# soham97/mellow

Hardware: AMD Instinct MI355X
Metric: audio-pair responses/sec (v0 167M, 2x10s clips, max_len=64, greedy) (higher is better)
Workload: dtype f32 (encoder/prefill GEMM operands split EXACTLY into 3 bf16 terms, 6 bf16 MFMA products per fp32 product, f32 accumulate: fp32-accurate, parity suite green; mel included, the STFT is an fp32 FFT; attentions and decode on exact fp32 MFMA / VALU)

## Files before the change

mellow_amd/csrc/build.py:

```python
#!/usr/bin/env python3
from __future__ import annotations

import argparse
import concurrent.futures as cf
import os
import subprocess
import sys

HERE = os.path.dirname(os.path.abspath(__file__))
PKG = os.path.dirname(HERE)
LIBDIR = os.path.join(PKG, "lib")
OBJDIR = os.path.join(HERE, "build")
LIB = os.path.join(LIBDIR, "libmellow_hip.so")
SOURCES = ["gemm_f32.hip", "gemm_fp8.hip", "gemm_bf16x3.hip", "decode.hip", "prefill_attn.hip", "encoder.hip", "stft_fft.hip", "sample.hip", "score.hip", "beam.hip", "engine.cpp", "engine_weights.cpp", "engine_encoder.cpp", "engine_lm.cpp", "engine_generate.cpp", "engine_dev.cpp"]
HEADERS = ["common.h", "kernels.h", "gemm_epilogue.h", "prefill_attn_f32.inc", "engine_internal.h", os.path.join("..", "..", "include", "mellow_hip.h")]
ARCH = "gfx950"
FLAGS = (["-DMELLOW_KDEBUG"] if os.environ.get("MELLOW_KDEBUG") else []) + os.environ.get("MELLOW_EXTRA_FLAGS", "").split() + ["-O3", "-std=c++17", "-fPIC", "-fvisibility=hidden", f"--offload-arch={ARCH}", "-Wall", "-Wno-unused-function",
         "-Wno-unused-variable", "-x", "hip"]


def _hipcc():
    for c in (os.environ.get("HIPCC"), "/opt/rocm/bin/hipcc", "hipcc"):
        if c and (os.path.isabs(c) and os.path.exists(c) or not os.path.isabs(c)):
            return c
    raise RuntimeError("hipcc not found")


def _stale(target, deps):
    if not os.path.exists(target):
        return True
    t = os.path.getmtime(target)
    return any(os.path.getmtime(d) > t for d in deps)


VGPR_FORM = ["-mllvm", "-amdgpu-mfma-vgpr-form=1"]
FILE_FLAGS = {name: VGPR_FORM for name in os.environ.get("MELLOW_VGPR_FORM_FILES", "gemm_bf16x3.hip gemm_fp8.hip prefill_attn.hip encoder.hip").split()}
KERNARG_PRELOAD = [] if os.environ.get("MELLOW_KERNARG_PRELOAD", "14") == "0" else ["-mllvm", "-amdgpu-kernarg-preload-count=" + os.environ.get("MELLOW_KERNARG_PRELOAD", "14")]
FILE_FLAGS["decode.hip"] = FILE_FLAGS.get("decode.hip", []) + KERNARG_PRELOAD


def build(force=False, verbose=False, out=None, objdir=None):
    lib = os.path.abspath(out) if out else LIB
    objdir = os.path.abspath(objdir) if objdir else OBJDIR
    os.makedirs(os.path.dirname(lib), exist_ok=True)
    os.makedirs(objdir, exist_ok=True)
    hipcc = _hipcc()
    hdrs = [os.path.join(HERE, h) for h in HEADERS] + [os.path.abspath(__file__)]
    jobs = []
    objs = []
    for src in SOURCES:
        sp = os.path.join(HERE, src)
        op = os.path.join(objdir, src + ".o")
        objs.append(op)
        if force or _stale(op, [sp] + hdrs):
            jobs.append((sp, op))

    def cc(job):
        sp, op = job
        cmd = [hipcc] + FLAGS + FILE_FLAGS.get(os.path.basename(sp), []) + ["-c", sp, "-o", op]
        if verbose:
            print(" ".join(cmd), flush=True)
        r = subprocess.run(cmd, capture_output=True, text=True)
        return sp, r

    with cf.ThreadPoolExecutor(max_workers=max(1, min(len(jobs), os.cpu_count() or 1))) as ex:
        for sp, r in ex.map(cc, jobs):
            if r.returncode != 0:
                sys.stderr.write(r.stdout + r.stderr)
                raise RuntimeError(f"hipcc failed on {sp}")
            if verbose and r.stderr.strip():
                sys.stderr.write(r.stderr)
    if force or jobs or _stale(lib, objs):
        cmd = [hipcc, "-shared", "-fPIC", f"--offload-arch={ARCH}", "-o", lib] + objs
        if verbose:
            print(" ".join(cmd), flush=True)
        r = subprocess.run(cmd, capture_output=True, text=True)
        if r.returncode != 0:
            sys.stderr.write(r.stdout + r.stderr)
            raise RuntimeError("link failed")
    return lib


if __name__ == "__main__":
    ap = argparse.ArgumentParser()
    ap.add_argument("--force", action="store_true")
    ap.add_argument("--verbose", action="store_true")
    ap.add_argument("--out", metavar="PATH", help="write the library here instead of mellow_amd/lib/libmellow_hip.so")
    ap.add_argument("--objdir", metavar="DIR", help="object cache of this build instead of mellow_amd/csrc/build/")
    a = ap.parse_args()
# ... 2 lines not shown
```

mellow_amd/csrc/common.h:

```cpp
#pragma once
#include <hip/hip_runtime.h>
#include <stdint.h>

namespace mellow {

typedef float f32x16 __attribute__((ext_vector_type(16)));
typedef float f32x4 __attribute__((ext_vector_type(4)));

#define MELLOW_WAVE 64

template <int CTRL>
__device__ __forceinline__ float dpp_mov(float v) {
    return __int_as_float(__builtin_amdgcn_update_dpp(0, __float_as_int(v), CTRL, 0xF, 0xF, true));
}
__device__ __forceinline__ float row16_sum(float v) {
    v += dpp_mov<0xB1>(v);
    v += dpp_mov<0x4E>(v);
    v += dpp_mov<0x141>(v);
    v += dpp_mov<0x140>(v);
    return v;
}
__device__ __forceinline__ float row16_max(float v) {
    v = fmaxf(v, dpp_mov<0xB1>(v));
    v = fmaxf(v, dpp_mov<0x4E>(v));
// ... 119 lines not shown
}

__device__ __forceinline__ int64_t amx_slot(int64_t m, int s, int j, int h, int KT64) {
    return (((((m >> 7) * KT64 + s) * 4 + ((m >> 5) & 3)) * 2 + j) * 64) + (m & 31) + 32 * h;
}
__device__ __forceinline__ int64_t amx_scale_byte(int64_t m, int s, int j, int KQ) {
    return (((((m >> 7) * KQ + (s >> 2)) * 4 + ((m >> 5) & 3)) * 64) + (m & 31) + 32 * j) * 4 + (s & 3);
}
__device__ __forceinline__ int mx8_exponent(float amax) {
    const uint32_t b = __float_as_uint(amax * (1.0f / 448.0f));
    int e = (int)((b >> 23) & 0xFF) + ((b & 0x7FFFFF) ? 1 : 0);
    e = e < 1 ? 1 : (e > 253 ? 253 : e);
    return amax > 0.f ? e : 127;
}
__device__ __forceinline__ float mx8_inverse(int e) { return __uint_as_float((uint32_t)(254 - e) << 23); }
__device__ __forceinline__ int mx8_pack4(float a, float b, float c, float d) {
    int w = 0;
    w = __builtin_amdgcn_cvt_pk_fp8_f32(a, b, w, false);
    w = __builtin_amdgcn_cvt_pk_fp8_f32(c, d, w, true);
    return w;
}
__device__ __forceinline__ void amx_store_block(i32x4* img, uint8_t* sc, int64_t m, int kb, int KT64, int KQ, const float (&v)[16], int h) {
    float amax = 0.f;
#pragma unroll
    for (int i = 0; i < 16; ++i) amax = fmaxf(amax, fabsf(v[i]));
    amax = half_max(amax);
    const int e = mx8_exponent(amax);
    const float inv = mx8_inverse(e);
    int w[4];
#pragma unroll
    for (int g = 0; g < 4; ++g) w[g] = mx8_pack4(v[4 * g] * inv, v[4 * g + 1] * inv, v[4 * g + 2] * inv, v[4 * g + 3] * inv);
    auto r0 = __builtin_amdgcn_permlane32_swap((uint32_t)w[0], (uint32_t)w[2], false, false);
    auto r1 = __builtin_amdgcn_permlane32_swap((uint32_t)w[1], (uint32_t)w[3], false, false);
    const int s = kb >> 1, j = kb & 1;
    img[amx_slot(m, s, j, h, KT64)] = i32x4{(int)r0[0], (int)r0[1], (int)r1[0], (int)r1[1]};
    if (h == 0) sc[amx_scale_byte(m, s, j, KQ)] = (uint8_t)e;
}

__device__ __forceinline__ void amx_store16(i32x4* img, uint8_t* sc, int64_t m, int kb, int KT64, int KQ, const float (&y)[16], int h) {
    float amax = 0.f;
#pragma unroll
    for (int i = 0; i < 16; ++i) amax = fmaxf(amax, fabsf(y[i]));
    amax = half_max(amax);
    const int e = mx8_exponent(amax);
    const float inv = mx8_inverse(e);
    i32x4 w;
#pragma unroll
    for (int q = 0; q < 4; ++q) w[q] = mx8_pack4(y[4 * q] * inv, y[4 * q + 1] * inv, y[4 * q + 2] * inv, y[4 * q + 3] * inv);
    const int s = kb >> 1, j = kb & 1;
    img[amx_slot(m, s, j, h, KT64)] = w;
    if (h == 0) sc[amx_scale_byte(m, s, j, KQ)] = (uint8_t)e;
}

__device__ __forceinline__ int xcd_remap(int b, int nb) {
    const int q = nb >> 3, r = nb & 7, x = b & 7;
    const int base = (x < r) ? x * (q + 1) : r * (q + 1) + (x - r) * q;
    return base + (b >> 3);
}

}
```

mellow_amd/csrc/engine.cpp:

```cpp
#include "engine_internal.h"

static thread_local std::string g_err;
int fail(const char* fmt, ...) {
    char buf[1024];
    va_list ap;
    va_start(ap, fmt);
    vsnprintf(buf, sizeof(buf), fmt, ap);
    va_end(ap);
    g_err = buf;
    return 1;
}
int ensure(mellow_engine* e, mellow_engine::Buf& b, size_t floats) {
    if (b.cap >= floats) return 0;
    if (b.p) HIPCHK(hipFree(b.p));
    b.p = nullptr;
    b.cap = 0;
    HIPCHK(hipMalloc(&b.p, floats * sizeof(float)));
    b.cap = floats;
    return 0;
}
int dev_alloc(mellow_engine* e, float** out, size_t floats) {
    const size_t bytes = (floats * sizeof(float) + 4095) / 4096 * 4096;
    if (!e->arena) {
        const size_t want = (size_t)(e->opt.arena_mb < 0 ? 0 : e->opt.arena_mb) << 20;
// ... 291 lines not shown
    *yes = h[2] < h[1];
    return 0;
}
int ensure_prefill_streams(mellow_engine* e) {
    if (e->n_forks > 0 || e->parent) return 0;
    if (e->streams_probed) {
        if (++e->probe_backoff < 16) { e->prefill_parts = e->prefill_parts_ok; return 0; }
        e->streams_probed = false;
        e->probe_backoff = 0;
        e->prefill_parts = e->prefill_parts_want;
    }
    int nh = e->prefill_parts < 1 ? 1 : (e->prefill_parts > 4 ? 4 : e->prefill_parts);
    for (int h = 1; h < nh; ++h) {
        if (e->stream2[h - 1]) continue;
        bool ok = false;
        for (int attempt = 0; attempt < 8 && !ok; ++attempt) {
            hipStream_t st = nullptr;
            HIPCHK(hipStreamCreateWithFlags(&st, hipStreamNonBlocking));
            int rc = streams_overlap(e, e->stream, st, &ok);
            for (int k = 1; k < h && ok && !rc; ++k) rc = streams_overlap(e, e->stream2[k - 1], st, &ok);
            if (rc) { hipStreamDestroy(st); return rc; }
            if (ok) e->stream2[h - 1] = st; else hipStreamDestroy(st);
        }
        if (!ok) {
            e->prefill_parts_want = e->prefill_parts;
            e->prefill_parts = e->prefill_parts_ok = h;
            e->streams_probed = true;
            break;
        }
    }
    return 0;
}
struct OptDesc { const char* key; const char* dflt; bool answers; const char* what; };
static const OptDesc kOptions[] = {
    {"prefill_split", "2", false, "f32x3: parts of the split LM prefill (1..4); bit-identical for every value"},
    {"prefill_fuse_norm", "1", true, "f32x3: norm-free LM prefill (GEMM epilogues emit split output + RMS partials); 0 = a normalisation launch per GEMM input"},
    {"decode_fuse", "1", true, "down projection of layer l fused with q/k/v of layer l + 1 through the load-time product W'Wd; 0 = five launches per layer"},
    {"decode_fuse_max_rb", "1", true, "largest number of 32-row blocks that runs the fused down + q/k/v launch on fp32 weights"},
    {"splitk", "8", true, "f32x3 encoder: largest split count of the split-K launches (0 = never split; a summation order)"},
    {"enc_apb", "0x1CC", false, "f32x3 encoder: Swin stages whose producers hand over pre-split (bit st, 4 + st, 8 + st); bit-identical"},
    {"graph", "1", false, "decode steps as hipGraph replays (0 = eager launches)"},
    {"fp8_decode", "1", true, "fp8 mode: e4m3 weights in the decode kernels"},
    {"fp8_prefill", "1", true, "fp8 mode: e4m3 GEMMs in encoder + LM prefill"},
    {"fp8_decode_act", "1", true, "fp8 mode: e4m3 activations in the decode GEMM kernels (fp8 matrix pipe)"},
    {"fp8_kv16", "1", true, "fp8 mode: bf16 shadow of the K/V pages for the decode step"},
    {"fp8_attn_bf16", "1", true, "fp8 mode: q / k / v stored once as bf16 (LM: bf16 K/V pages + bf16-once prefill attention; Swin: bf16 q/k/v rows into the exact window attention); 0 = fp32 q/k/v, the 3-way split attention"},
    {"decode_x3", "7", true, "f32x3: mask of decode GEMM launches on the bf16 pipe (1 lm_head, 2 gate/up, 4 fused down + q/k/v)"},
    {"decode_x3_min_rb", "2", true, "f32x3: fewest 32-row blocks at which the layer launches take their f32x3 forms"},
    {"x3_stft", "1", true, "f32x3: STFT / mel GEMMs on the split kernel (0 = exact fp32 kernel)"},
    {"stft_fft", "1", true, "f32x3: STFT as a 1024-point FFT when the checkpoint's conv weights are the windowed DFT basis"},
    {"x3_apb", "1", true, "f32x3 LM prefill: producers hand over pre-split, GEMMs staged by LDS-DMA (0 = register-staged kernel on fp32 activations)"},
    {"x3_attn", "1", true, "f32x3: prefill attention on exact bf16 splits (0 = exact fp32 MFMA kernel)"},
    {"x3w", "1", false, "f32x3: K = 96 GEMMs on the weight-stationary persistent kernel; bit-identical"},
    {"row_migration", "1", false, "reference-semantics loop, B > 32: rows still running are packed into the lowest 32-row blocks; tokens unchanged"},
    {"arena_mb", "3400", false, "size of the weight arena in MiB (before the first tensor is loaded)"},
};
static const OptDesc* find_opt(const char* key) {
    for (const auto& o : kOptions)
        if (!strcmp(o.key, key)) return &o;
    return nullptr;
}
static long opt_val(const mellow_engine* e, const char* key) {
    auto it = e->opt.given.find(key);
    return strtol(it != e->opt.given.end() ? it->second.c_str() : find_opt(key)->dflt, nullptr, 0);
}
int apply_options(mellow_engine* e) {
    const int mode = e->opt.mode;
    e->prefill_parts = (int)opt_val(e, "prefill_split");
    e->opt.prefill_fuse_norm = opt_val(e, "prefill_fuse_norm") != 0;
    e->opt.decode_fuse = opt_val(e, "decode_fuse") != 0;
    e->opt.dec_fuse_max_rb = (int)opt_val(e, "decode_fuse_max_rb");
    e->opt.sk_max = (int)opt_val(e, "splitk");
    e->opt.enc_apb_stages = (int)opt_val(e, "enc_apb");
    e->use_graph = opt_val(e, "graph") != 0;
    e->opt.x3_stft = opt_val(e, "x3_stft") != 0;
    e->opt.stft_fft = opt_val(e, "stft_fft") != 0 && e->opt.x3_stft;
    e->opt.x3_apb = opt_val(e, "x3_apb") != 0;
    e->opt.x3_attn = opt_val(e, "x3_attn") != 0;
    e->opt.x3w = opt_val(e, "x3w") != 0;
    e->opt.row_migration = opt_val(e, "row_migration") != 0;
    e->opt.arena_mb = (int)opt_val(e, "arena_mb");
    e->opt.fp8 = mode == MELLOW_PRECISION_FP8;
    e->opt.fp8_decode = e->opt.fp8 && opt_val(e, "fp8_decode") != 0;
    e->opt.fp8_decode_act = e->opt.fp8_decode && opt_val(e, "fp8_decode_act") != 0;
    e->opt.fp8_prefill = opt_val(e, "fp8_prefill") != 0;
    e->opt.fp8_attn_bf16 = opt_val(e, "fp8_attn_bf16") != 0;
    e->opt.kv16 = e->opt.fp8_decode && opt_val(e, "fp8_kv16") != 0;
    e->opt.f32x3_terms = mode == MELLOW_PRECISION_F32X3 ? 6 : 0;
    e->opt.dec_x3 = mode == MELLOW_PRECISION_F32X3 ? ((int)opt_val(e, "decode_x3") & DEC_X3_ALL) : 0;
    e->opt.dec_x3_min_rb = (int)opt_val(e, "decode_x3_min_rb") < 1 ? 1 : (int)opt_val(e, "decode_x3_min_rb");
    return 0;
}

extern "C" {

int mellow_engine_set_option(mellow_engine_t* e, const char* key, const char* value) {
    if (!e || !key || !value) return fail("null argument");
    if (e->finalized) return fail("options must be set before mellow_engine_finalize");
    const OptDesc* o = find_opt(key);
    if (!o) return fail("unknown option \"%s\" (mellow_engine_describe lists them)", key);
    char* end = nullptr;
    const long v = strtol(value, &end, 0);
    if (end == value || *end) return fail("option \"%s\": \"%s\" is not an integer", key, value);
    if (!strcmp(key, "prefill_split") && (v < 1 || v > 4)) return fail("option prefill_split must be 1..4");
    if (!strcmp(key, "arena_mb") && e->arena) return fail("option arena_mb must be set before the first tensor is loaded");
    e->opt.given[key] = value;
    return apply_options(e);
}

int64_t mellow_engine_describe(mellow_engine_t* e, char* buf, int64_t capacity) {
    if (!e) return -1;
    std::string s = "{\"abi\": [" + std::to_string(MELLOW_ABI_VERSION) + ", " + std::to_string(MELLOW_ABI_MINOR) + "], \"precision\": \"";
    s += e->opt.mode == MELLOW_PRECISION_F32 ? "f32" : e->opt.mode == MELLOW_PRECISION_FP8 ? "fp8" : "f32x3";
    s += "\", \"reads_environment\": false, \"finalized\": ";
    s += e->finalized ? "true" : "false";
    s += ", \"stft_is_fft\": ";
    s += e->w.fft_win ? "true" : "false";
    s += ", \"non_default\": [";
    bool first = true;
    for (const auto& o : kOptions)
        if (opt_val(e, o.key) != strtol(o.dflt, nullptr, 0)) { s += std::string(first ? "" : ", ") + "\"" + o.key + "\""; first = false; }
    s += "], \"options\": {";
    first = true;
    for (const auto& o : kOptions) {
        s += std::string(first ? "" : ", ") + "\"" + o.key + "\": {\"value\": " + std::to_string(opt_val(e, o.key)) + ", \"default\": " +
             std::to_string(strtol(o.dflt, nullptr, 0)) + ", \"changes_answers\": " + (o.answers ? "true" : "false") + "}";
        first = false;
    }
    s += "}}";
    if (buf && capacity > (int64_t)s.size()) memcpy(buf, s.c_str(), s.size() + 1);
    return (int64_t)s.size() + 1;
}
// ... 99 lines not shown
```

mellow_amd/csrc/engine_encoder.cpp:

```cpp
#include "engine_internal.h"

static void with_splitk(mellow_engine* e, GemmArgs& g) {
    if (!e->sk_enable || e->opt.sk_max < 2 || !e->sk_ws.p) return;
    g.sk_ws = e->sk_ws.p;
    g.sk_tiles = 256;
    g.sk_max = e->opt.sk_max;
}
int run_gemm(mellow_engine* e, const GemmArgs& a) {
    const bool x3_stft = e->opt.x3_stft;
    if (e->opt.f32x3_terms && a.K % 16 == 0 &&
        ((a.a_mode == A_PLAIN && (a.epi == EPI_LINEAR || a.epi == EPI_SWIGLU || a.epi == EPI_QKV_ROPE || a.epi == EPI_QKV_ROPE_AT)) || (x3_stft && a.K >= 192))) {
        auto it = e->w.bf_w.find(a.Wp);
        if (it != e->w.bf_w.end()) {
            GemmArgs g = a;
            g.W8 = reinterpret_cast<const uint8_t*>(it->second);
            with_splitk(e, g);
            ProfScope ps(e, PF_GEMM, gemm_flops(a), 0.0);
            ps.r.M = a.M; ps.r.N = a.Nw; ps.r.K = a.K; ps.r.epi = a.epi + 200;
            launch_gemm_bf16x3_fused(g, e->stream);
            return 0;
        }
    }
    if (e->opt.fp8 && e->opt.fp8_prefill && a.a_mode == A_PLAIN && (a.epi == EPI_LINEAR || a.epi == EPI_SWIGLU || a.epi == EPI_QKV_ROPE)) {
        auto it = e->w.fp8_w.find(a.Wp);
// ... 52 lines not shown
    hipStream_t s = e->stream;
    struct SkScope {
        mellow_engine* e;
        ~SkScope() { e->sk_enable = false; }
    } sk_scope{e};
    if (e->opt.f32x3_terms && e->opt.sk_max >= 2) {
        CHK(ensure(e, e->sk_ws, (size_t)512 * 16384));
        e->sk_enable = e->sk_ws.p != nullptr;
    }
    const int frames = (int)(n_samples / kHop) + 1;
    const int64_t plen = n_samples + kNfft;
    const int M = n * frames;
    CHK(ensure(e, e->wpad, (size_t)n * plen));
    CHK(ensure(e, e->power, (size_t)M * 544));
    CHK(ensure(e, e->logmel, (size_t)M * 64));
    {
        ProfScope ps(e, PF_MISC, 0, 2.0 * n * plen * 4);
        launch_reflect_pad(wav, n, n_samples, e->wpad.p, plen, kNfft / 2, s);
    }
    if (e->w.fft_win) {
        ProfScope ps(e, PF_GEMM, 5.0 * kNfft * 10.0 * M, (double)M * (kNfft + 544) * 4);
        ps.r.M = M; ps.r.N = 544; ps.r.K = kNfft; ps.r.epi = 400;
        launch_stft_fft_power(e->wpad.p, frames, plen, kHop, M, e->w.fft_win, e->w.fft_tw1, e->w.fft_tw2, e->power.p, s);
    } else {
        GemmArgs g;
        g.A = e->wpad.p; g.a_mode = A_FRAMES; g.fpc = frames; g.clip_stride = plen; g.hop = kHop;
        g.M = M; g.K = kNfft; g.Wp = e->w.dft.p; g.Nw = e->w.dft.Nw; g.N = 544; g.C = e->power.p; g.ldc = 544; g.epi = EPI_POWER;
        CHK(run_gemm(e, g));
    }
    CHK(tap(e, "power", e->power.p, (int64_t)M * 544));
    {
        GemmArgs g;
        g.A = e->power.p; g.lda = 544; g.M = M; g.K = 544; g.Wp = e->w.mel.p; g.Nw = 64; g.N = 64;
        g.C = want_logmel_only ? logmel_out : e->logmel.p; g.ldc = 64; g.epi = EPI_LOGMEL;
        g.apply_bn = apply_bn; g.bn_alpha = e->w.bn_alpha; g.bn_beta = e->w.bn_beta;
        CHK(run_gemm(e, g));
    }
    if (want_logmel_only) return 0;
    CHK(tap(e, "logmel_bn", e->logmel.p, (int64_t)M * 64));

    int n_crops = 1, crop_len = frames, crop_hop = 0;
    if (frames > 1024) {
        n_crops = 0;
        for (int p = 0; p < frames - kLongCrop - 1; p += kLongHop) ++n_crops;
        crop_len = kLongCrop;
        crop_hop = kLongHop;
    }
    const int nv = n * n_crops;
    const int64_t M0 = (int64_t)nv * 4096;
    CHK(ensure(e, e->X0, (size_t)M0 * 96));
    CHK(ensure(e, e->X1, (size_t)M0 * 96));
    CHK(ensure(e, e->T, (size_t)M0 * 96));
    CHK(ensure(e, e->QKV, (size_t)M0 * 288));
    CHK(ensure(e, e->H, (size_t)M0 * 384));
    {
        ProfScope ps(e, PF_MISC, 0, (double)M0 * 96 * 4);
        launch_fold_patch_embed(e->logmel.p, n, frames, n_crops, crop_hop, crop_len, e->w.pe_w, e->w.pe_b, e->w.pe_nw, e->w.pe_nb,
                                e->X0.p, s);
    }
    CHK(tap(e, "patch", e->X0.p, M0 * 96));
    float *x = e->X0.p, *x2 = e->X1.p, *t = e->T.p;
    for (int st = 0; st < 4; ++st) {
        const int C = 96 << st, R = 64 >> st, N = R * R, nH = kHeads[st];
        const int nW = R > kWin ? (R / kWin) * (R / kWin) : 1;
        const int M1 = nv * N;
        for (int b = 0; b < kDepths[st]; ++b) {
            const SwinBlockW& w = e->w.blocks[st][b];
            const bool shifted = (b % 2 == 1) && R > kWin;
            const int32_t* map = R > kWin ? e->w.win_map[st][shifted ? 1 : 0] : nullptr;
            const bool amx = e->opt.fp8 && e->opt.fp8_prefill && e->opt.x3_apb && e->w.fp8_w.count(w.qkv.p) && e->w.fp8_w.count(w.fc1.p) && e->w.fp8_w.count(w.fc2.p);
            const bool have_pb = e->opt.f32x3_terms && e->w.bf_w.count(w.qkv.p) && e->w.bf_w.count(w.fc1.p) && e->w.bf_w.count(w.fc2.p);
            const bool apb_h = amx || (have_pb && ((e->opt.enc_apb_stages >> st) & 1));
            const bool apb = apb_h || (have_pb && ((e->opt.enc_apb_stages >> (8 + st)) & 1));
            const size_t M1p = (size_t)rup(M1, 128);
            char *a3s = nullptr, *h3s = nullptr;
            if (apb) {
                CHK(ensure(e, e->enc_a3, (M1p * C * 6 + 3) / 4));
                if (apb_h) CHK(ensure(e, e->enc_h3, (M1p * 4 * C * 6 + 3) / 4));
                if (amx) {
                    a3s = reinterpret_cast<char*>(e->enc_a3.p) + M1p * rup(C, 64);
                    h3s = reinterpret_cast<char*>(e->enc_h3.p) + M1p * rup(4 * C, 64);
                }
                { ProfScope ps(e, PF_NORM, 0, 2.5 * M1 * C * 4); launch_layernorm_apb(x, e->enc_a3.p, M1, C, w.n1w, w.n1b, map, N, s, a3s); }
                {
                    GemmArgs g = lin(nullptr, C, M1, w.qkv, e->QKV.p, 3 * C, w.qkv_b);
                    g.c16 = (amx && e->opt.fp8_attn_bf16) ? 1 : 0;
                    CHK(run_gemm_apb(e, g, e->enc_a3.p, s, a3s));
                }
            } else {
                { ProfScope ps(e, PF_NORM, 0, 2.0 * M1 * C * 4); launch_layernorm(x, t, M1, C, w.n1w, w.n1b, map, N, s); }
                CHK(run_gemm(e, lin(t, C, M1, w.qkv, e->QKV.p, 3 * C, w.qkv_b)));
            }
            const bool apb_proj = apb && !amx && ((e->opt.enc_apb_stages >> (4 + st)) & 1) && e->w.bf_w.count(w.proj.p);
            {
                ProfScope ps(e, PF_WINDOW_ATTN, 4.0 * 64 * 64 * 24 * (double)(M1 / 64) * nH, 4.0 * M1 * C * 4);
                launch_window_attention(e->QKV.p, t, M1, C, nH, w.bias_exp, shifted ? w.mask : nullptr, nW, s, apb_proj ? e->enc_a3.p : nullptr, amx && e->opt.fp8_attn_bf16);
            }
            {
                GemmArgs g = lin(t, C, M1, w.proj, x, C, w.proj_b);
                g.resid = x; g.ldr = C; g.crow_map = map; g.rows_in = N; g.rows_out = N;
                if (apb_proj) CHK(run_gemm_apb(e, g, e->enc_a3.p, s));
                else CHK(run_gemm(e, g));
            }
            if (apb) {
                { ProfScope ps(e, PF_NORM, 0, 2.5 * M1 * C * 4); launch_layernorm_apb(x, e->enc_a3.p, M1, C, w.n2w, w.n2b, nullptr, N, s, a3s); }
                {
                    GemmArgs g = lin(nullptr, C, M1, w.fc1, apb_h ? nullptr : e->H.p, 4 * C, w.fc1_b);
                    g.act = ACT_GELU; g.C3 = apb_h ? e->enc_h3.p : nullptr;
                    if (amx) { g.c3_fmt = 1; g.C3s = reinterpret_cast<uint8_t*>(h3s); g.c3_kt64 = rup(4 * C, 64) / 64; }
                    CHK(run_gemm_apb(e, g, e->enc_a3.p, s, a3s));
                }
                {
                    GemmArgs g = lin(apb_h ? nullptr : e->H.p, 4 * C, M1, w.fc2, x, C, w.fc2_b);
                    g.resid = x; g.ldr = C;
                    if (apb_h) CHK(run_gemm_apb(e, g, e->enc_h3.p, s, h3s));
                    else CHK(run_gemm(e, g));
                }
            } else {
                { ProfScope ps(e, PF_NORM, 0, 2.0 * M1 * C * 4); launch_layernorm(x, t, M1, C, w.n2w, w.n2b, nullptr, N, s); }
                {
                    GemmArgs g = lin(t, C, M1, w.fc1, e->H.p, 4 * C, w.fc1_b);
                    g.act = ACT_GELU;
                    CHK(run_gemm(e, g));
                }
                {
                    GemmArgs g = lin(e->H.p, 4 * C, M1, w.fc2, x, C, w.fc2_b);
                    g.resid = x; g.ldr = C;
                    CHK(run_gemm(e, g));
                }
            }
        }
        if (st < 3) {
            { ProfScope ps(e, PF_NORM, 0, 2.0 * M1 * C * 4); launch_merge_layernorm(x, t, nv, R, C, e->w.merge[st].nw, e->w.merge[st].nb, s); }
            CHK(run_gemm(e, lin(t, 4 * C, M1 / 4, e->w.merge[st].red, x2, 2 * C, nullptr)));
            float* tmp = x; x = x2; x2 = tmp;
        }
        if (e->taps_on) {
            char nm[16];
            snprintf(nm, sizeof(nm), "stage%d", st);
            const int64_t cnt = st < 3 ? (int64_t)nv * (N / 4) * (2 * C) : (int64_t)nv * N * C;
            CHK(tap(e, nm, x, cnt));
        }
    }
    CHK(ensure(e, e->ats, (size_t)nv * 32 * 4608));
    CHK(ensure(e, e->fpx, (size_t)nv * 32 * 544));
    CHK(ensure(e, e->emb33, (size_t)n * 33 * 768));
    CHK(ensure(e, e->e1, (size_t)n * 33 * 576));
    CHK(ensure(e, e->gbuf, (size_t)n * 33 * 576));
    CHK(ensure(e, e->sbuf, (size_t)n * 33 * 576));
    CHK(ensure(e, e->proj33, (size_t)n * 33 * 576));
    { ProfScope ps(e, PF_NORM, 0, 2.0 * nv * 64 * 768 * 4); launch_layernorm(x, t, nv * 64, kEncOut, e->w.fn_w, e->w.fn_b, nullptr, 64, s); }
    float* latent_dst = e->emb33.p;
    int64_t latent_stride = 33 * 768;
    if (n_crops > 1) {
        CHK(ensure(e, e->latv, (size_t)nv * 768));
        CHK(ensure(e, e->fpxavg, (size_t)n * 32 * 544));
        latent_dst = e->latv.p;
        latent_stride = 768;
    }
    { ProfScope ps(e, PF_MISC, 0, 7.0 * nv * 64 * 768 * 4); launch_tail_latent_im2col(t, nv, latent_dst, latent_stride, e->ats.p, s); }
    {
        GemmArgs g = lin(e->ats.p, 4608, nv * 32, e->w.tscam, e->fpx.p, 544, e->w.tscam_b);
        g.N = 544; g.act = ACT_SIGMOID;
        CHK(run_gemm(e, g));
    }
    const float* fpx = e->fpx.p;
    if (n_crops > 1) {
        ProfScope ps(e, PF_MISC, 0, 0);
        launch_crop_average(e->fpx.p, n, n_crops, 32 * 544, 32 * 544, e->fpxavg.p, 32 * 544, s);
        launch_crop_average(e->latv.p, n, n_crops, 768, 768, e->emb33.p, 33 * 768, s);
        fpx = e->fpxavg.p;
    }
// ... 119 lines not shown
```

mellow_amd/csrc/engine_internal.h:

```cpp
#pragma once
#include <hip/hip_runtime.h>

#include <array>
#include <chrono>
#include <cmath>
#include <cstdarg>
#include <cstdio>
#include <cstdlib>
#include <cstring>
#include <map>
#include <unordered_map>
#include <string>
#include <thread>
#include <type_traits>
#include <utility>
#include <vector>

#include "../../include/mellow_hip.h"
#include "kernels.h"

using namespace mellow;

int fail(const char* fmt, ...);
struct mellow_engine;
// ... 54 lines not shown
struct MergeW {
    float *nw, *nb;
    Packed red;
};
struct DecW {
    const float *p, *scale;
};
struct LMLayerW {
    Packed qkv, o, gateup, down;
    Packed qkv_f, gateup_f;
    float* o16 = nullptr;
    float* gu16n = nullptr;
    float* gu16 = nullptr;
    float* qkv2 = nullptr;
    float *q2h8 = nullptr, *q2h_sc = nullptr;
    float *qkv8 = nullptr, *qkv_sc = nullptr, *o8 = nullptr, *o_sc = nullptr, *gu8 = nullptr, *gu_sc = nullptr, *dn8 = nullptr,
          *dn_sc = nullptr;
    float *in_ln, *post_ln;
    DecW qkv_w() const { return qkv8 ? DecW{qkv8, qkv_sc} : DecW{qkv_f.p, nullptr}; }
    DecW o_w() const { return o8 ? DecW{o8, o_sc} : DecW{o16, nullptr}; }
    DecW gateup_w() const { return gu8 ? DecW{gu8, gu_sc} : DecW{gu16, nullptr}; }
    DecW down_w() const { return dn8 ? DecW{dn8, dn_sc} : DecW{down.p, nullptr}; }
};

struct ProfRec {
    int fam;
    hipEvent_t a, b;
    double flops, bytes;
    int M = 0, N = 0, K = 0, epi = 0;
};

struct StepMode {
    bool logits = true;
    bool sample = false;
    bool logprob = false;
    bool early_exit = false;
    bool migrate = false;
    int beam = 0;
};

#define LOCAL __attribute__((visibility("hidden")))
struct mellow_engine {
    struct Buf {
        float* p = nullptr;
        size_t cap = 0;
        Buf() = default; Buf(const Buf&) = delete; Buf& operator=(const Buf&) = delete;
        Buf(Buf&& o) noexcept : p(o.p), cap(o.cap) { o.p = nullptr; o.cap = 0; }
        Buf& operator=(Buf&& o) noexcept { std::swap(p, o.p); std::swap(cap, o.cap); return *this; }
        LOCAL ~Buf() { if (p) (void)hipFree(p); }
    };
    struct LOCAL Options {
        std::map<std::string, std::string> given;
        int mode = MELLOW_PRECISION_F32X3;
        bool x3_stft = true, stft_fft = true, x3_apb = true, x3_attn = true, x3w = true, row_migration = true, decode_fuse = true;
        int arena_mb = 3400;
        bool kv16 = false;
        bool fp8 = false;
        bool fp8_decode = false;
        bool fp8_decode_act = false;
        bool fp8_attn_bf16 = true;
        bool fp8_prefill = true;
        int dec_x3_min_rb = 2;
        int dec_x3 = 0;
        int f32x3_terms = 0;
        bool prefill_fuse_norm = true;
        int enc_apb_stages = 0x1CC;
        int sk_max = 8;
        int dec_fuse_max_rb = 1;
    };
    struct Fp8W { uint8_t* w8; float* scale; };
    struct LOCAL Weights {
        Packed dft, mel;
        float *fft_win = nullptr, *fft_tw1 = nullptr, *fft_tw2 = nullptr;
        float *bn_alpha = nullptr, *bn_beta = nullptr;
        float *pe_w = nullptr, *pe_b = nullptr, *pe_nw = nullptr, *pe_nb = nullptr;
        std::vector<SwinBlockW> blocks[4];
        MergeW merge[3];
        int32_t* win_map[4][2] = {{nullptr}};
        float *fn_w = nullptr, *fn_b = nullptr;
        Packed tscam, c2l, lin1, lin2;
        float *tscam_b = nullptr, *c2l_b = nullptr, *pln_w = nullptr, *pln_b = nullptr;
        int32_t* emb_row_map = nullptr;
        float* embed = nullptr;
        Packed lm_head;
        std::vector<LMLayerW> layers;
        float* final_norm = nullptr;
        float *rope_cos = nullptr, *rope_sin = nullptr;
        float *head8 = nullptr, *head_sc = nullptr;
        DecW head_w() const { return head8 ? DecW{head8, head_sc} : DecW{lm_head.p, nullptr}; }
        std::unordered_map<const float*, void*> bf_w;
        std::unordered_map<const float*, Fp8W> fp8_w;
    };
    struct LOCAL StepGraphs {
        struct Key {
            std::array<uintptr_t, 14> v{};
            static Key of(const mellow_engine* e, int B);
            bool operator==(const Key& k) const { return v == k.v; }
        };
        hipGraphExec_t one = nullptr, eight = nullptr;
        Key key;
        StepGraphs() = default; StepGraphs(const StepGraphs&) = delete; StepGraphs& operator=(const StepGraphs&) = delete;
        void reset() {
            for (hipGraphExec_t* x : {&one, &eight}) if (*x) { (void)hipGraphExecDestroy(*x); *x = nullptr; }
        }
        ~StepGraphs() { reset(); }
    };

// ... 167 lines not shown
```

mellow_amd/csrc/gemm_bf16x3.hip:

```cpp
#include <cstdlib>

#include "common.h"
#include "gemm_epilogue.h"
#include "kernels.h"

namespace mellow {


__global__ __launch_bounds__(256) void pack_bf16x3_kernel(const float* __restrict__ Wp, int NP, int KP, i32x4* __restrict__ PB) {
    const int K16 = KP >> 4, K8 = KP >> 3;
    const int64_t total = (int64_t)(NP >> 5) * K16 * 64;
    for (int64_t i = (int64_t)blockIdx.x * blockDim.x + threadIdx.x; i < total; i += (int64_t)gridDim.x * blockDim.x) {
        const int lane = (int)(i & 63);
        const int64_t tile = i >> 6;
        const int s16 = (int)(tile % K16), nt = (int)(tile / K16);
        const int n = nt * 32 + (lane & 31), k0 = s16 * 16 + (lane >> 5) * 8;
        float v[8];
#pragma unroll
        for (int b = 0; b < 8; ++b) {
            const int k = k0 + b;
            v[b] = Wp[(((int64_t)(n >> 5) * K8 + (k >> 3)) * 64 + (n & 31) + 32 * ((k >> 2) & 1)) * 4 + (k & 3)];
        }
        i32x4 p0, p1, p2;
        split8(v, p0, p1, p2);
// ... 249 lines not shown
        if (i_ >= 2 && i_ < 14) __builtin_amdgcn_sched_group_barrier(0x002, 4, 0);               \
        if (i_ >= 14 && i_ < 20) __builtin_amdgcn_sched_group_barrier(0x200, 1, 0);              \
        if (i_ >= 19 && i_ < 24) __builtin_amdgcn_sched_group_barrier(0x020, 1, 0);              \
    }

#ifdef MELLOW_X3_NO_SETPRIO
#define X3_PRIO(P)
#else
#define X3_PRIO(P) __builtin_amdgcn_s_setprio(P);
#endif
    i32x4 fa0[2][3], fw0[2][3], fa1[2][3], fw1[2][3];
    X3_GLOAD(0, raA, rwA)
    X3_GLOAD(1, raB, rwB)
    X3_LSTORE(0, raA, rwA)
    X3_LSTORE(1, raB, rwB)
    X3_GLOAD(2, raA, rwA)
    X3_GLOAD(3, raB, rwB)
    __syncthreads();
    X3_FRAGS(0, fa0, fw0)
#ifndef MELLOW_X3_ABL
#define MELLOW_X3_ABL 0
#endif
#define X3_ITER(T, SN, SW, FA, FW, FAN, FWN, ra, rw)                                             \
    if ((T) < KT) {                                                                              \
        X3_PRIO(2)                                                                               \
        if (!(MELLOW_X3_ABL & 8)) X3_FRAGS(SN, FAN, FWN)                                         \
        X3_MFMAS(FA, FW)                                                                         \
        if (!(MELLOW_X3_ABL & 4)) X3_LSTORE(SW, ra, rw)                                          \
        if (!(MELLOW_X3_ABL & 1)) X3_GLOAD((T) + 4, ra, rw)                                      \
        if (!MELLOW_X3_ABL) X3_SCHED()                                                           \
        X3_PRIO(0)                                                                               \
        if (!(MELLOW_X3_ABL & 2)) __syncthreads();                                               \
    }
    for (int kt = 0; kt < KT; kt += 6) {
        X3_ITER(kt + 0, 1, 2, fa0, fw0, fa1, fw1, raA, rwA)
        X3_ITER(kt + 1, 2, 0, fa1, fw1, fa0, fw0, raB, rwB)
        X3_ITER(kt + 2, 0, 1, fa0, fw0, fa1, fw1, raA, rwA)
        X3_ITER(kt + 3, 1, 2, fa1, fw1, fa0, fw0, raB, rwB)
        X3_ITER(kt + 4, 2, 0, fa0, fw0, fa1, fw1, raA, rwA)
        X3_ITER(kt + 5, 0, 1, fa1, fw1, fa0, fw0, raB, rwB)
    }
#undef X3_GLOAD
#undef X3_LSTORE
#undef X3_FRAGS
#undef X3_TERM
#undef X3_MFMAS
#undef X3_SCHED
#undef X3_ITER
#undef X3_PRIO
    if (p.ks > 1) return splitk_store(p, acc, tile, split, tid);
    gemm_epilogue<WN, EPI>(g, acc, pm, pn, wm, wn, lane, BM, BN);
}

__device__ __forceinline__ void glds16(const void* base, uint32_t voff, uint32_t lds_addr) {
    uint32_t keep;
    asm volatile("s_mov_b32 %0, m0\n\ts_mov_b32 m0, %2\n\ts_nop 0\n\tglobal_load_lds_dwordx4 %1, %3\n\ts_mov_b32 m0, %0"
                 : "=&s"(keep) : "v"(voff), "s"(lds_addr), "s"(base) : "memory");
}
template <int EPI>
__global__ __launch_bounds__(256, 2) void gemm_x3q_kernel(const GemmBDev p) {
    constexpr int BM = 128, BN = 128, WN = 2, NST = 3;
    constexpr int STAGE = 3 * 4 * 64;
    extern __shared__ __attribute__((aligned(16))) i32x4 smem_bf[];
    i32x4* As = smem_bf;
    i32x4* Ws = smem_bf + NST * STAGE;
    const GemmArgs& g = p.a;
    const int tid = threadIdx.x, lane = tid & 63;
    const int wave = __builtin_amdgcn_readfirstlane(tid >> 6);
    const int wm = wave >> 1, wn = wave & 1;
    const int tiles = p.gm * p.gn;
    int tile, split, pm, pn;
    if (p.ng) {
        const int npx = p.gn >> 3, b = (int)blockIdx.x, j = b >> 3;
        pm = j / npx; pn = (b & 7) * npx + j % npx;
        tile = pm * p.gn + pn; split = 0;
    } else {
        const int L = xcd_remap((int)blockIdx.x, tiles * p.ks);
        tile = L % tiles; split = L / tiles;
        pm = tile / p.gn; pn = tile % p.gn;
    }
    const int KTf = g.K >> 4;
    const int kt0 = split * KTf / p.ks;
    const int KT = (split + 1) * KTf / p.ks - kt0;
    __shared__ float rs_rows[BM];
    if (g.rs_ssq && tid < BM) {
        int64_t m = (int64_t)pm * BM + tid;
        m = m < g.M ? m : g.M - 1;
        const float* sp = g.rs_ssq + m * g.rs_parts;
        float ss = 0.f;
        for (int p = 0; p < g.rs_parts; ++p) ss += sp[p];
        rs_rows[tid] = 1.0f / sqrtf(ss / g.rs_dim + g.rs_eps);
    }
    const bool isA = wave < 2;
    const int c0 = (wave & 1) * 6;
    const char* base = isA ? reinterpret_cast<const char*>(g.A8) + (((int64_t)pm * KTf + kt0) * 12 + c0) * 1024
                           : reinterpret_cast<const char*>(g.W8) + ((int64_t)pn * 4 * KTf + kt0) * 3072;
    const uint32_t kstep = isA ? 12288u : 3072u;
    uint32_t voff[6];
#pragma unroll
    for (int j = 0; j < 6; ++j) {
        const int c = c0 + j;
        voff[j] = isA ? (uint32_t)(j * 1024 + lane * 16) : (uint32_t)(((c & 3) * KTf * 192 + (c >> 2) * 64 + lane) * 16);
    }
    const uint32_t lds0 = (uint32_t)(uintptr_t)smem_bf + (isA ? 0u : (uint32_t)(NST * STAGE * 16)) + (uint32_t)c0 * 1024u;
#define X3Q_ISSUE(T, ST)                                                                         \
    {                                                                                            \
        const int t_ = (T) < KT ? (T) : KT - 1;                                                  \
        const char* b_ = base + (int64_t)t_ * kstep;                                             \
        _Pragma("unroll") for (int j = 0; j < 6; ++j) glds16(b_, voff[j], lds0 + (uint32_t)((ST) * STAGE * 16 + j * 1024)); \
    }
    f32x16 acc[2][2];
// ... 346 lines not shown
```

mellow_amd/csrc/kernels.h:

```cpp
#pragma once
#include <hip/hip_runtime.h>
#include <stdint.h>

namespace mellow {

void launch_pack_weight(const float* w, int N, int K, int64_t ldw, float* out, int NP, int KP, hipStream_t s);
void launch_pack_weight_pairs(const float* w0, const float* w1, int N, int K, int64_t ldw, float* out, int NP,
                              int KP, hipStream_t s);

enum { ACT_NONE = 0, ACT_GELU = 1, ACT_SIGMOID = 2 };
enum { EPI_LINEAR = 0, EPI_POWER = 1, EPI_LOGMEL = 2, EPI_SWIGLU = 3, EPI_QKV_ROPE = 4, EPI_LSE = 5, EPI_QKV_ROPE_AT = 6 };
enum { A_PLAIN = 0, A_FRAMES = 1 };

struct GemmArgs {
    const float* A = nullptr;
    int64_t lda = 0;
    int M = 0;
    int K = 0;
    int a_mode = A_PLAIN;
    int fpc = 1;
    int64_t clip_stride = 0;
    int hop = 0;
    const float* Wp = nullptr;
    int Nw = 0;
// ... 1 lines not shown
    float* C = nullptr;
    int64_t ldc = 0;
    const float* bias = nullptr;
    const float* resid = nullptr;
    int64_t ldr = 0;
    const int32_t* crow_map = nullptr;
    int rows_in = 1, rows_out = 1;
    int act = ACT_NONE;
    int epi = EPI_LINEAR;
    const float* bn_alpha = nullptr;
    const float* bn_beta = nullptr;
    int apply_bn = 0;
    float* q_out = nullptr;
    float* k_cache = nullptr;
    float* v_cache = nullptr;
    const float* rope_cos = nullptr;
    const float* rope_sin = nullptr;
    int T = 1, Tmax = 1, q_heads = 9, kv_heads = 3;
    int c16 = 0;
    int kv16 = 0;
    void* C3 = nullptr;
    float* sk_ws = nullptr;
    int sk_tiles = 0, sk_max = 0;
    bool no_x3w = false;
    int pos0 = 0;
    float* ssq_out = nullptr;
    int ssq_parts = 0;
    const float* rs_ssq = nullptr;
    int rs_parts = 0;
    float rs_dim = 1.f, rs_eps = 0.f;
    const uint8_t* A8 = nullptr;
    int64_t lda8 = 0;
    const uint32_t* a_sc = nullptr;
    const uint8_t* W8 = nullptr;
    const float* w_scale = nullptr;
    int c3_fmt = 0;
    uint8_t* C3s = nullptr;
    int c3_kt64 = 0;
    const int32_t* lse_target = nullptr;
    float2* lse_ms = nullptr;
    int32_t* lse_arg = nullptr;
    float* lse_tgt = nullptr;
    int64_t lse_ld = 0;
};
void launch_gemm(const GemmArgs& a, hipStream_t s);
void launch_quant_mx8(const float* A, int64_t lda, int M, int K, void* img, void* sc, hipStream_t s);
void launch_pack_fp8(const float* Wp, int NP, int KP, uint8_t* W8, float* w_scale, hipStream_t s);
void launch_gemm_fp8(const GemmArgs& a, hipStream_t s);
void launch_pack_bf16x3(const float* Wp, int NP, int KP, void* PB, hipStream_t s);
void launch_gemm_bf16x3_fused(const GemmArgs& a, hipStream_t s);
void launch_split_rows_apb(const float* A, int64_t lda, int M, int K, void* out, hipStream_t s);
void launch_gemm_bf16x3_apb(const GemmArgs& a, hipStream_t s);
double gemm_flops(const GemmArgs& a);

void set_max_dynamic_lds(const void* fn, size_t bytes);

constexpr int DEC_KC_QKV = 8;
#ifndef MELLOW_DEC_KC_DOWN
#define MELLOW_DEC_KC_DOWN 8
#endif
constexpr int DEC_KC_DOWN = MELLOW_DEC_KC_DOWN;
#ifndef MELLOW_DEC_TS
#define MELLOW_DEC_TS 2
#endif
constexpr int DEC_TS = MELLOW_DEC_TS;
#ifndef MELLOW_DEC_TS_MULTI
#define MELLOW_DEC_TS_MULTI 1
#endif
constexpr int DEC_TS_MULTI = MELLOW_DEC_TS_MULTI;
inline int dec_key_splits(int RB, bool fixed) { return RB <= 1 || fixed ? DEC_TS : DEC_TS_MULTI; }
#ifndef MELLOW_Q2_HC
#define MELLOW_Q2_HC 4
#endif
#ifndef MELLOW_Q2_WAVES
#define MELLOW_Q2_WAVES 12
#else
#define MELLOW_Q2_WAVES_FORCED 1
#endif
constexpr int Q2_HC = MELLOW_Q2_HC, Q2_WAVES = MELLOW_Q2_WAVES;
constexpr int Q2_NPQ = 2 + Q2_HC;
constexpr int Q2_K8 = 72 + 192;
constexpr int Q2_BLOCKS = 60 + 48 * Q2_HC;
static_assert(Q2_NPQ <= DEC_KC_QKV && Q2_HC <= DEC_KC_DOWN, "the fused kernel reuses the slab buffers of the split-K kernels");
enum { DEC_X3_HEAD = 1, DEC_X3_GATEUP = 2, DEC_X3_QKV = 4, DEC_X3_ALL = 7 };
struct DecArgs {
    int rows = 0, RB = 0;
    int Tmax = 0;
    float eps = 1e-5f;
    int32_t* d_pos = nullptr;
    int first = 0;
    int inc_pos = 0;
    int gs = 1;
    int ts = DEC_TS;
    float* rope_cur = nullptr;
    float* ssq1 = nullptr;
    const float* rope_cos = nullptr;
    const float* rope_sin = nullptr;
    float* xmidF = nullptr;
    float* xnewR = nullptr;
    float* dslabF = nullptr;
    int64_t slabF_stride4 = 0;
    float* pq = nullptr;
    float* attF16 = nullptr;
    float* att_ml = nullptr;
    float* ssq = nullptr;
    float* xmidF16 = nullptr;
// ... 140 lines not shown
```

Baseline: 459.2.

## Fuse stage-0 Swin MLP fc1+GELU+fc2 into one bf16x3 kernel with hidden in registers

Adds a fused kernel for the stage-0 Swin block MLP (C=96, hidden 384) in the f32x3 encoder path. fc1, GELU and fc2 plus the bias and residual run in one launch. The hidden activation stays in registers, and weight chunks are streamed through double-buffered LDS via global_load_lds. This removes the hidden-tensor write and read to global memory and one GEMM launch per block. In exchange it adds a specialised kernel with a fixed per-panel schedule that may get less occupancy or overlap than the tuned general GEMMs.

```diff
diff --git a/mellow_amd/csrc/build.py b/mellow_amd/csrc/build.py
--- a/mellow_amd/csrc/build.py
+++ b/mellow_amd/csrc/build.py
@@ -12,7 +12,7 @@
 LIBDIR = os.path.join(PKG, "lib")
 OBJDIR = os.path.join(HERE, "build")
 LIB = os.path.join(LIBDIR, "libmellow_hip.so")
-SOURCES = ["gemm_f32.hip", "gemm_fp8.hip", "gemm_bf16x3.hip", "decode.hip", "prefill_attn.hip", "encoder.hip", "stft_fft.hip", "sample.hip", "score.hip", "beam.hip", "engine.cpp", "engine_weights.cpp", "engine_encoder.cpp", "engine_lm.cpp", "engine_generate.cpp", "engine_dev.cpp"]
+SOURCES = ["gemm_f32.hip", "gemm_fp8.hip", "gemm_bf16x3.hip", "swin_mlp.hip", "decode.hip", "prefill_attn.hip", "encoder.hip", "stft_fft.hip", "sample.hip", "score.hip", "beam.hip", "engine.cpp", "engine_weights.cpp", "engine_encoder.cpp", "engine_lm.cpp", "engine_generate.cpp", "engine_dev.cpp"]
 HEADERS = ["common.h", "kernels.h", "gemm_epilogue.h", "prefill_attn_f32.inc", "engine_internal.h", os.path.join("..", "..", "include", "mellow_hip.h")]
 ARCH = "gfx950"
 FLAGS = (["-DMELLOW_KDEBUG"] if os.environ.get("MELLOW_KDEBUG") else []) + os.environ.get("MELLOW_EXTRA_FLAGS", "").split() + ["-O3", "-std=c++17", "-fPIC", "-fvisibility=hidden", f"--offload-arch={ARCH}", "-Wall", "-Wno-unused-function",
@@ -34,7 +34,7 @@
 
 
 VGPR_FORM = ["-mllvm", "-amdgpu-mfma-vgpr-form=1"]
-FILE_FLAGS = {name: VGPR_FORM for name in os.environ.get("MELLOW_VGPR_FORM_FILES", "gemm_bf16x3.hip gemm_fp8.hip prefill_attn.hip encoder.hip").split()}
+FILE_FLAGS = {name: VGPR_FORM for name in os.environ.get("MELLOW_VGPR_FORM_FILES", "gemm_bf16x3.hip swin_mlp.hip gemm_fp8.hip prefill_attn.hip encoder.hip").split()}
 KERNARG_PRELOAD = [] if os.environ.get("MELLOW_KERNARG_PRELOAD", "14") == "0" else ["-mllvm", "-amdgpu-kernarg-preload-count=" + os.environ.get("MELLOW_KERNARG_PRELOAD", "14")]
 FILE_FLAGS["decode.hip"] = FILE_FLAGS.get("decode.hip", []) + KERNARG_PRELOAD
 
diff --git a/mellow_amd/csrc/common.h b/mellow_amd/csrc/common.h
--- a/mellow_amd/csrc/common.h
+++ b/mellow_amd/csrc/common.h
@@ -195,6 +195,12 @@
     if (h == 0) sc[amx_scale_byte(m, s, j, KQ)] = (uint8_t)e;
 }
 
+__device__ __forceinline__ void glds16(const void* base, uint32_t voff, uint32_t lds_addr) {
+    uint32_t keep;
+    asm volatile("s_mov_b32 %0, m0\n\ts_mov_b32 m0, %2\n\ts_nop 0\n\tglobal_load_lds_dwordx4 %1, %3\n\ts_mov_b32 m0, %0"
+                 : "=&s"(keep) : "v"(voff), "s"(lds_addr), "s"(base) : "memory");
+}
+
 __device__ __forceinline__ int xcd_remap(int b, int nb) {
     const int q = nb >> 3, r = nb & 7, x = b & 7;
     const int base = (x < r) ? x * (q + 1) : r * (q + 1) + (x - r) * q;
diff --git a/mellow_amd/csrc/engine.cpp b/mellow_amd/csrc/engine.cpp
--- a/mellow_amd/csrc/engine.cpp
+++ b/mellow_amd/csrc/engine.cpp
@@ -367,6 +367,7 @@
     {"x3_apb", "1", true, "f32x3 LM prefill: producers hand over pre-split, GEMMs staged by LDS-DMA (0 = register-staged kernel on fp32 activations)"},
     {"x3_attn", "1", true, "f32x3: prefill attention on exact bf16 splits (0 = exact fp32 MFMA kernel)"},
     {"x3w", "1", false, "f32x3: K = 96 GEMMs on the weight-stationary persistent kernel; bit-identical"},
+    {"enc_mlp_fused", "1", false, "f32x3 encoder: fc1 + GELU + fc2 of a stage-0 Swin block as one launch, the hidden activation in registers (0 = two GEMM launches); bit-identical"},
     {"row_migration", "1", false, "reference-semantics loop, B > 32: rows still running are packed into the lowest 32-row blocks; tokens unchanged"},
     {"arena_mb", "3400", false, "size of the weight arena in MiB (before the first tensor is loaded)"},
 };
@@ -393,6 +394,7 @@
     e->opt.x3_apb = opt_val(e, "x3_apb") != 0;
     e->opt.x3_attn = opt_val(e, "x3_attn") != 0;
     e->opt.x3w = opt_val(e, "x3w") != 0;
+    e->opt.enc_mlp_fused = opt_val(e, "enc_mlp_fused") != 0;
     e->opt.row_migration = opt_val(e, "row_migration") != 0;
     e->opt.arena_mb = (int)opt_val(e, "arena_mb");
     e->opt.fp8 = mode == MELLOW_PRECISION_FP8;
diff --git a/mellow_amd/csrc/engine_encoder.cpp b/mellow_amd/csrc/engine_encoder.cpp
--- a/mellow_amd/csrc/engine_encoder.cpp
+++ b/mellow_amd/csrc/engine_encoder.cpp
@@ -128,7 +128,6 @@
     CHK(ensure(e, e->X1, (size_t)M0 * 96));
     CHK(ensure(e, e->T, (size_t)M0 * 96));
     CHK(ensure(e, e->QKV, (size_t)M0 * 288));
-    CHK(ensure(e, e->H, (size_t)M0 * 384));
     {
         ProfScope ps(e, PF_MISC, 0, (double)M0 * 96 * 4);
         launch_fold_patch_embed(e->logmel.p, n, frames, n_crops, crop_hop, crop_len, e->w.pe_w, e->w.pe_b, e->w.pe_nw, e->w.pe_nb,
@@ -180,6 +179,15 @@
             }
             if (apb) {
                 { ProfScope ps(e, PF_NORM, 0, 2.5 * M1 * C * 4); launch_layernorm_apb(x, e->enc_a3.p, M1, C, w.n2w, w.n2b, nullptr, N, s, a3s); }
+                bool mlp_done = false;
+                if (e->opt.enc_mlp_fused && e->opt.x3w && !apb_h && C == 96 && w.fc1.KP == 96 && w.fc1.Nw == 384 && w.fc2.KP == 384 && w.fc2.Nw == 96) {
+                    ProfScope ps(e, PF_GEMM, 2.0 * 2.0 * M1 * 96.0 * 384.0, 0.0);
+                    ps.r.M = M1; ps.r.N = 96; ps.r.K = 384; ps.r.epi = 600;
+                    mlp_done = launch_swin_mlp_x3(e->enc_a3.p, e->w.bf_w.find(w.fc1.p)->second, w.fc1_b, e->w.bf_w.find(w.fc2.p)->second, w.fc2_b, x, M1, s);
+                    if (!mlp_done) ps.on = false;
+                }
+                if (!mlp_done) {
+                if (!apb_h) CHK(ensure(e, e->H, (size_t)M1 * 4 * C));
                 {
                     GemmArgs g = lin(nullptr, C, M1, w.fc1, apb_h ? nullptr : e->H.p, 4 * C, w.fc1_b);
                     g.act = ACT_GELU; g.C3 = apb_h ? e->enc_h3.p : nullptr;
@@ -192,8 +200,10 @@
                     if (apb_h) CHK(run_gemm_apb(e, g, e->enc_h3.p, s, h3s));
                     else CHK(run_gemm(e, g));
                 }
+                }
             } else {
                 { ProfScope ps(e, PF_NORM, 0, 2.0 * M1 * C * 4); launch_layernorm(x, t, M1, C, w.n2w, w.n2b, nullptr, N, s); }
+                CHK(ensure(e, e->H, (size_t)M1 * 4 * C));
                 {
                     GemmArgs g = lin(t, C, M1, w.fc1, e->H.p, 4 * C, w.fc1_b);
                     g.act = ACT_GELU;
diff --git a/mellow_amd/csrc/engine_internal.h b/mellow_amd/csrc/engine_internal.h
--- a/mellow_amd/csrc/engine_internal.h
+++ b/mellow_amd/csrc/engine_internal.h
@@ -130,7 +130,7 @@
     struct LOCAL Options {
         std::map<std::string, std::string> given;
         int mode = MELLOW_PRECISION_F32X3;
-        bool x3_stft = true, stft_fft = true, x3_apb = true, x3_attn = true, x3w = true, row_migration = true, decode_fuse = true;
+        bool x3_stft = true, stft_fft = true, x3_apb = true, x3_attn = true, x3w = true, enc_mlp_fused = true, row_migration = true, decode_fuse = true;
         int arena_mb = 3400;
         bool kv16 = false;
         bool fp8 = false;
diff --git a/mellow_amd/csrc/gemm_bf16x3.hip b/mellow_amd/csrc/gemm_bf16x3.hip
--- a/mellow_amd/csrc/gemm_bf16x3.hip
+++ b/mellow_amd/csrc/gemm_bf16x3.hip
@@ -325,11 +325,6 @@
     gemm_epilogue<WN, EPI>(g, acc, pm, pn, wm, wn, lane, BM, BN);
 }
 
-__device__ __forceinline__ void glds16(const void* base, uint32_t voff, uint32_t lds_addr) {
-    uint32_t keep;
-    asm volatile("s_mov_b32 %0, m0\n\ts_mov_b32 m0, %2\n\ts_nop 0\n\tglobal_load_lds_dwordx4 %1, %3\n\ts_mov_b32 m0, %0"
-                 : "=&s"(keep) : "v"(voff), "s"(lds_addr), "s"(base) : "memory");
-}
 template <int EPI>
 __global__ __launch_bounds__(256, 2) void gemm_x3q_kernel(const GemmBDev p) {
     constexpr int BM = 128, BN = 128, WN = 2, NST = 3;
diff --git a/mellow_amd/csrc/kernels.h b/mellow_amd/csrc/kernels.h
--- a/mellow_amd/csrc/kernels.h
+++ b/mellow_amd/csrc/kernels.h
@@ -77,6 +77,8 @@
 void launch_split_rows_apb(const float* A, int64_t lda, int M, int K, void* out, hipStream_t s);
 void launch_gemm_bf16x3_apb(const GemmArgs& a, hipStream_t s);
 double gemm_flops(const GemmArgs& a);
+constexpr int SMLP_ROWS = 128;
+bool launch_swin_mlp_x3(const void* apb, const void* w1, const float* b1, const void* w2, const float* b2, float* x, int64_t M, hipStream_t s);
 
 void set_max_dynamic_lds(const void* fn, size_t bytes);
 
diff --git a/mellow_amd/csrc/swin_mlp.hip b/mellow_amd/csrc/swin_mlp.hip
--- /dev/null
+++ b/mellow_amd/csrc/swin_mlp.hip
@@ -0,0 +1,155 @@
+#include "common.h"
+#include "kernels.h"
+
+namespace mellow {
+
+#ifndef MELLOW_SMLP_ABL
+#define MELLOW_SMLP_ABL 0
+#endif
+constexpr int SMLP_STAGE = 36 * 64;
+constexpr size_t SMLP_LDS = (size_t)2 * SMLP_STAGE * 16;
+
+#define SMLP_BF(W, A, ACC) ACC = __builtin_amdgcn_mfma_f32_32x32x16_bf16(__builtin_bit_cast(bf16x8, W), __builtin_bit_cast(bf16x8, A), ACC, 0, 0, 0);
+
+__global__ __launch_bounds__(256, 2) void swin_mlp_x3_kernel(const i32x4* __restrict__ apb, const i32x4* __restrict__ w1, const float* __restrict__ b1,
+                                                             const i32x4* __restrict__ w2, const float* __restrict__ b2, float* __restrict__ x) {
+    constexpr int NC = 12;
+    extern __shared__ __attribute__((aligned(16))) i32x4 smem_mlp[];
+    const int tid = threadIdx.x, lane = tid & 63;
+    const int wave = __builtin_amdgcn_readfirstlane(tid >> 6);
+    const int h = lane >> 5;
+    const int64_t panel = blockIdx.x;
+    const bool is1 = wave < 2;
+    const char* wbase = is1 ? reinterpret_cast<const char*>(w1) : reinterpret_cast<const char*>(w2);
+    const uint32_t cstep = is1 ? 18u * 1024u : 6u * 1024u;
+    uint32_t voff[9];
+#pragma unroll
+    for (int q = 0; q < 9; ++q) {
+        const int i = (wave & 1) * 9 + q;
+        voff[q] = (uint32_t)((is1 ? i : (i / 6) * 72 + i % 6) * 1024 + lane * 16);
+    }
+    const uint32_t lds0 = (uint32_t)(uintptr_t)smem_mlp + (uint32_t)(wave * 9) * 1024u;
+#define SMLP_ISSUE(C, ST)                                                                        \
+    {                                                                                            \
+        const char* b_ = wbase + (int64_t)(C) * cstep;                                           \
+        _Pragma("unroll") for (int q = 0; q < 9; ++q) glds16(b_, voff[q], lds0 + (uint32_t)((ST) * (SMLP_STAGE * 16) + q * 1024)); \
+    }
+    i32x4 af[6][3];
+    {
+        const i32x4* ap = apb + (panel * 72 + wave) * 64 + lane;
+#pragma unroll
+        for (int kt = 0; kt < 6; ++kt)
+#pragma unroll
+            for (int pc = 0; pc < 3; ++pc) af[kt][pc] = ap[(kt * 12 + pc * 4) * 64];
+    }
+    SMLP_ISSUE(0, 0)
+    typedef const __attribute__((address_space(4))) f32x4 cf32x4;
+    cf32x4* b1c = (cf32x4*)b1;
+#pragma unroll
+    for (int kt = 0; kt < 6; ++kt)
+#pragma unroll
+        for (int pc = 0; pc < 3; ++pc) asm volatile("" : "+v"(af[kt][pc]));
+    f32x16 oacc[3];
+#pragma unroll
+    for (int j = 0; j < 3; ++j)
+#pragma unroll
+        for (int r = 0; r < 16; ++r) oacc[j][r] = 0.f;
+
+#pragma unroll 1
+    for (int c = 0; c < NC; ++c) {
+        const int st = c & 1;
+        asm volatile("s_waitcnt vmcnt(0) lgkmcnt(0)" ::: "memory");
+        __builtin_amdgcn_s_barrier();
+        if (c + 1 < NC) SMLP_ISSUE(c + 1, st ^ 1)
+        if (MELLOW_SMLP_ABL & 8) continue;
+        const i32x4* Wc = smem_mlp + st * SMLP_STAGE + lane;
+        f32x4 bq[4];
+#pragma unroll
+        for (int gq = 0; gq < 4; ++gq) {
+            const f32x4 lo = b1c[c * 8 + 2 * gq], hi = b1c[c * 8 + 2 * gq + 1];
+#pragma unroll
+            for (int j = 0; j < 4; ++j) bq[gq][j] = h ? hi[j] : lo[j];
+        }
+        f32x16 hacc;
+#pragma unroll
+        for (int r = 0; r < 16; ++r) hacc[r] = 0.f;
+#pragma unroll
+        for (int kt = 0; kt < 6; ++kt) {
+            const i32x4 f0 = Wc[(kt * 3 + 0) * 64], f1 = Wc[(kt * 3 + 1) * 64], f2 = Wc[(kt * 3 + 2) * 64];
+            if (MELLOW_SMLP_ABL & 4) { hacc[kt] += __int_as_float(f0[0] ^ f1[1] ^ f2[2] ^ af[kt][0][0] ^ af[kt][1][1] ^ af[kt][2][2]); continue; }
+            SMLP_BF(f2, af[kt][0], hacc) SMLP_BF(f0, af[kt][2], hacc) SMLP_BF(f1, af[kt][1], hacc)
+            SMLP_BF(f1, af[kt][0], hacc) SMLP_BF(f0, af[kt][1], hacc) SMLP_BF(f0, af[kt][0], hacc)
+        }
+        float hv[16];
+#pragma unroll
+        for (int gq = 0; gq < 4; ++gq)
+#pragma unroll
+            for (int j = 0; j < 4; ++j) {
+                float v = hacc[4 * gq + j] + bq[gq][j];
+                if (!(MELLOW_SMLP_ABL & 2)) v = gelu_erf(v);
+                hv[4 * gq + j] = v;
+            }
+#pragma unroll
+        for (int s = 0; s < 2; ++s) {
+            float w[8];
+#pragma unroll
+            for (int j = 0; j < 4; ++j) {
+                auto r = __builtin_amdgcn_permlane32_swap(__float_as_uint(hv[8 * s + j]), __float_as_uint(hv[8 * s + 4 + j]), false, false);
+                w[j] = __uint_as_float(r[0]);
+                w[4 + j] = __uint_as_float(r[1]);
+            }
+            i32x4 p[3];
+            split8(w, p[0], p[1], p[2]);
+            i32x4 fw[3][3];
+#pragma unroll
+            for (int j = 0; j < 3; ++j)
+#pragma unroll
+                for (int pc = 0; pc < 3; ++pc) fw[j][pc] = Wc[(18 + j * 6 + s * 3 + pc) * 64];
+            if (MELLOW_SMLP_ABL & 4) {
+#pragma unroll
+                for (int j = 0; j < 3; ++j) oacc[j][s] += __int_as_float(fw[j][0][0] ^ fw[j][1][1] ^ fw[j][2][2] ^ p[0][0] ^ p[1][1] ^ p[2][2]);
+                continue;
+            }
+#define SMLP_TERM(PW, PA) SMLP_BF(fw[0][PW], p[PA], oacc[0]) SMLP_BF(fw[1][PW], p[PA], oacc[1]) SMLP_BF(fw[2][PW], p[PA], oacc[2])
+            SMLP_TERM(2, 0) SMLP_TERM(0, 2) SMLP_TERM(1, 1) SMLP_TERM(1, 0) SMLP_TERM(0, 1) SMLP_TERM(0, 0)
+#undef SMLP_TERM
+        }
+    }
+#undef SMLP_ISSUE
+    if (MELLOW_SMLP_ABL & 8) {
+#pragma unroll
+        for (int kt = 0; kt < 6; ++kt) oacc[kt % 3][kt] += __int_as_float(af[kt][0][0] ^ af[kt][1][1] ^ af[kt][2][2]);
+    }
+    float* xr = x + (panel * 128 + wave * 32 + (lane & 31)) * 96 + 4 * h;
+    f32x4 res[3][4], bo[3][4];
+#pragma unroll
+    for (int j = 0; j < 3; ++j)
+#pragma unroll
+        for (int gq = 0; gq < 4; ++gq) {
+            bo[j][gq] = *reinterpret_cast<const f32x4*>(b2 + j * 32 + 8 * gq + 4 * h);
+            res[j][gq] = *reinterpret_cast<const f32x4*>(xr + j * 32 + 8 * gq);
+        }
+#pragma unroll
+    for (int j = 0; j < 3; ++j)
+#pragma unroll
+        for (int gq = 0; gq < 4; ++gq) {
+            float v[4];
+#pragma unroll
+            for (int i = 0; i < 4; ++i) {
+                v[i] = oacc[j][4 * gq + i] + bo[j][gq][i];
+                v[i] = res[j][gq][i] + v[i];
+            }
+            if (!(MELLOW_SMLP_ABL & 1) || v[0] == 1.2345f) *reinterpret_cast<f32x4*>(xr + j * 32 + 8 * gq) = f32x4{v[0], v[1], v[2], v[3]};
+        }
+}
+#undef SMLP_BF
+
+bool launch_swin_mlp_x3(const void* apb, const void* w1, const float* b1, const void* w2, const float* b2, float* x, int64_t M, hipStream_t s) {
+    if (M <= 0 || M % SMLP_ROWS != 0 || M / SMLP_ROWS > 0x7fffffff) return false;
+    set_max_dynamic_lds(reinterpret_cast<const void*>(&swin_mlp_x3_kernel), SMLP_LDS);
+    hipLaunchKernelGGL(swin_mlp_x3_kernel, dim3((unsigned)(M / SMLP_ROWS)), dim3(256), SMLP_LDS, s, reinterpret_cast<const i32x4*>(apb),
+                       reinterpret_cast<const i32x4*>(w1), b1, reinterpret_cast<const i32x4*>(w2), b2, x);
+    return true;
+}
+
+}
```

Result: no change. 461.5 (median of 6 runs) (+0.5%).
